# davidfang00/opticalflowdiffusion

Hardware: AMD Instinct MI355X
Metric: UNet denoise steps/sec @ 2x436x1024 flow, bs=16 (higher is better)
Workload: dtype bf16

## Files before the change

### opticalflowdiffusion_amd/csrc/blocks.h

```cpp
#pragma once
#include "common.h"

namespace ofd {

struct MlpDesc {
    const float* weight;
    const float* bias;
    int n_out;
    int offset;
};

struct FcFuse { const float* w; const float* b; float* out; };
bool conv_fc_fuse_supported(const ofd_conv_args* a, int out_dim);
int conv_forward_impl(const ofd_conv_args* a, hipStream_t s, int pool2 = 0, const bf16_t* residual_b = nullptr, const FcFuse* fc = nullptr);
bool conv_pool2_supported(const ofd_conv_args* a);
bool conv_residual_b_supported(const ofd_conv_args* a);
int k_wt_transpose(const bf16_t* w, bf16_t* wt, int taps, int Cin, int Cout, hipStream_t s);
int k_conv_wgrad(const ofd_conv_args* a, const bf16_t* dy, float* dw, hipStream_t s, float* dbias = nullptr);
int k_conv7_wgrad(const bf16_t* x16, const bf16_t* dy, float* dw, int B, int H, int W, hipStream_t s, float* dbias = nullptr, int channels = 16);
int k_channel_sum(const bf16_t* dy, float* out, size_t npix, int C, hipStream_t s);
int k_wgrad_finish(const float* acc, const float* w_raw, float* dst, int Cout, int Cin, int Cin_pad, int ksize, float ws_eps, int unshuffle,
                   int accumulate, hipStream_t s);
int k_grad_scatter(const bf16_t* D, int Ctot, int ch_off, bf16_t* dst, int C, int B, int H, int W, int mode, int p1, int p2, int accumulate,
                   hipStream_t s);

struct ofd_weight_prep_desc {
    const float* w;
    void* out;
    int Cout, Cin, Cin_pad, ksize;
    float ws_eps;
    int unshuffle;
    int block0;
};
int k_conv_weight_prep_batched(const ofd_weight_prep_desc* d_descs, int n, int total_blocks, hipStream_t s);
int k_wt_transpose_batched(const ofd_weight_prep_desc* d_descs, int n, int total_blocks, hipStream_t s);
int k_pack_input(const float* x, int Cx, const float* cond, int Cc, bf16_t* out, int B, int H, int W, hipStream_t s, int cpad = 16, int ax = 0, int ac = 0);
int k_time_mlp(const int64_t* t, const float* w1, const float* b1, const float* w2, const float* b2, float* temb,
               float* temb_silu, int B, int dim, hipStream_t s);
int k_block_mlp(const float* temb_silu, const MlpDesc* descs, int n_desc, float* ss, int B, int tdim, int ss_stride, hipStream_t s);
int k_gn_finalize(const float* partial, int B, int H, int W, int C, const float* gamma, const float* beta, const float* ss,
                  int ss_stride, int ss_offset, float* a_out, float* s_out, hipStream_t s, float* stats_out = nullptr);
int k_resblock_out(const bf16_t* h, const float* a, const float* sft, const bf16_t* x, bf16_t* out, int B, int H, int W, int C, hipStream_t s);
int k_layernorm_c(const bf16_t* x, const float* g, const bf16_t* res, bf16_t* out, size_t npix, int C, float eps, hipStream_t s);
int la_parts(int B, int n);
int k_linear_attention_core(const bf16_t* qkv, float* partial, float* ctx, bf16_t* out, int B, int n, hipStream_t s, float* ml_out = nullptr,
                            const bf16_t* wo = nullptr, const float* bo = nullptr, bf16_t* o2 = nullptr, int C = 0);
int la_fused_blocks(int n, int B, int C = 64);
int la_fwd_parts(int B, int n);
int k_linear_attention_fused_train(const bf16_t* x, const bf16_t* wq, const bf16_t* wkv, const bf16_t* woutp, const float* bias, const float* g_pre,
                                   const float* g2, float* partial, bf16_t* ctxfrag, float* ctx, float* ml, bf16_t* xn, bf16_t* qkv, bf16_t* o2,
                                   bf16_t* y, int B, int n, int C, float eps_pre, float eps_post, hipStream_t s);
int k_la_weight_prep(const float* wqkv, const float* g, const float* wout, bf16_t* wq, bf16_t* wkv, bf16_t* woutp, int C, hipStream_t s);
int k_linear_attention_fused(const bf16_t* x, const bf16_t* wq, const bf16_t* wkv, const bf16_t* woutp, const float* bias, const float* g2,
                             float* partial, bf16_t* ctxfrag, bf16_t* y, int B, int n, int C, float eps_pre, float eps_post, hipStream_t s);
int k_flash_attention(const bf16_t* qkv, bf16_t* out, int B, int n, hipStream_t s, float* lse = nullptr);
int k_final_conv(const bf16_t* x, const float* w, const float* bias, float* out, int B, int H, int W, int C, int out_dim, hipStream_t s, int out_mode = 0,
                 float out_div = 1.0f);
int k_nhwc_to_nchw(const bf16_t* x, float* out, int B, int H, int W, int C, hipStream_t s);
int k_nchw_to_nhwc(const float* x, bf16_t* out, int B, int H, int W, int C, hipStream_t s);

int k_affine_silu(const bf16_t* h, const float* a, const float* s, bf16_t* out, int B, int H, int W, int C, hipStream_t st);
size_t gn_bwd_workspace_floats(int B, int H, int W, int C);
int k_gn_silu_backward(const bf16_t* g, const bf16_t* h, const float* a, const float* s, const float* stats, const float* gamma,
                       const float* beta, const float* ss, int ss_stride, int ss_offset, bf16_t* dh, float* dgamma, float* dbeta, float* dss,
                       float* workspace, int B, int H, int W, int C, hipStream_t st, float* dconv_bias = nullptr);
int k_layernorm_c_bwd(const bf16_t* x, const float* gw, const bf16_t* dy, bf16_t* dx, float* dg, size_t npix, int C, float eps, int accumulate,
                      hipStream_t st, const bf16_t* extra = nullptr);
int k_final_conv_bwd(const bf16_t* x, const float* w, const float* dy, bf16_t* dx, float* dw, float* db, int B, int H, int W, int C, int out_dim,
                     hipStream_t st, const float* bias = nullptr, int out_mode = 0, float out_div = 1.0f);
int k_conv7_dgrad(const bf16_t* dy, const bf16_t* wt, int cin_pad, float* dx, int cx, int B, int H, int W, float scale, hipStream_t s);
int k_block_mlp_bwd(const float* dss, const float* temb_silu, const float* weight, int n_out, int offset, float* dweight, float* dbias, float* dts,
                    int B, int tdim, int ss_stride, hipStream_t st);
int k_time_mlp_bwd(const int64_t* t, const float* temb, const float* dts, const float* w1, const float* b1, const float* w2, float* dw1, float* db1,
                   float* dw2, float* db2, float* scratch, int B, int dim, hipStream_t st);
int k_grad_add(bf16_t* dst, const bf16_t* src, size_t elems, int accumulate, hipStream_t st);

size_t la_bwd_workspace_floats(int B, int n);
int k_linear_attention_core_bwd(const bf16_t* qkv, const bf16_t* dout, const float* ctx, const float* ml, bf16_t* dqkv, float* workspace, int B, int n,
                                hipStream_t s);
int k_linear_attention_block_bwd(const bf16_t* qkv, const bf16_t* do2, const float* ctx, const float* ml, float* workspace, int B, int n, hipStream_t s,
                                 const bf16_t* xn, const bf16_t* wt, float* dw, bf16_t* dxn, const bf16_t* wo_fwd, const bf16_t* wo_t, float* dwo,
                                 float* dbo, const bf16_t* wq);
int k_flash_attention_bwd(const bf16_t* qkv, const bf16_t* o, const bf16_t* dout, const float* lse, bf16_t* dqkv, float* delta, int B, int n,
                          hipStream_t s);

}
```

### opticalflowdiffusion_amd/csrc/la_fused.hip

```cpp
#include <cstdlib>
#include <type_traits>
#include "blocks.h"
#include "la_common.h"

namespace ofd {

template <int C>
struct XRaw {
    u32x4 v[C / 16];
};

template <int C>
__device__ __forceinline__ void load_raw_x(const bf16_t* __restrict__ xrow, XRaw<C>& r, int half) {
#pragma unroll
    for (int s = 0; s < C / 16; ++s) r.v[s] = *(const u32x4*)(xrow + 16 * s + 8 * half);
}

template <int N16, class At>
__device__ __forceinline__ void la_stage(unsigned char* dst, const bf16_t* __restrict__ src, int tid, At at) {
    static_assert(N16 % (8 * 256) == 0, "whole turns of eight units per thread");
    for (int i0 = tid; i0 < N16; i0 += 8 * 256) {
        uint4 v[8];
#pragma unroll
        for (int k = 0; k < 8; ++k) v[k] = ((const uint4*)src)[at(i0 + k * 256)];
#pragma unroll
        for (int k = 0; k < 8; ++k) ((uint4*)dst)[i0 + k * 256] = v[k];
    }
}
template <int N16>
__device__ __forceinline__ void la_stage(unsigned char* dst, const bf16_t* __restrict__ src, int tid) {
    la_stage<N16>(dst, src, tid, [](int i) { return i; });
}

typedef __bf16 la_bf16x2 __attribute__((ext_vector_type(2)));
template <int C>
__device__ __forceinline__ void norm_stats(const XRaw<C>& r, float eps, float& rstd, float& off) {
    const la_bf16x2 one = __builtin_bit_cast(la_bf16x2, 0x3f803f80u);
    float s1 = 0.0f, s2 = 0.0f;
#pragma unroll
    for (int s = 0; s < C / 16; ++s)
#pragma unroll
        for (int j = 0; j < 4; ++j) {
            const la_bf16x2 w = __builtin_bit_cast(la_bf16x2, (uint32_t)r.v[s][j]);
            s1 = __builtin_amdgcn_fdot2_f32_bf16(w, one, s1, false);
            s2 = __builtin_amdgcn_fdot2_f32_bf16(w, w, s2, false);
        }
    s1 += __shfl_xor(s1, 32, 64);
    s2 += __shfl_xor(s2, 32, 64);
    const float mean = s1 * (1.0f / C);
    const float var = fmaxf(__builtin_fmaf(-mean, mean, s2 * (1.0f / C)), 0.0f);
    rstd = rsqrtf(var + eps);
    off = -mean * rstd;
}
template <int C>
__device__ __forceinline__ void norm_x(const XRaw<C>& r, float eps, bf16x8 (&xs)[C / 16]) {
    float rstd, off;
    norm_stats<C>(r, eps, rstd, off);
#pragma unroll
    for (int s = 0; s < C / 16; ++s)
#pragma unroll
        for (int j = 0; j < 4; ++j) {
            const uint32_t w = r.v[s][j];
            xs[s][2 * j] = (__bf16)__builtin_fmaf(bf2f((bf16_t)(w & 0xffffu)), rstd, off);
            xs[s][2 * j + 1] = (__bf16)__builtin_fmaf(bf2f((bf16_t)(w >> 16)), rstd, off);
// ... 56 lines not shown
    }
    __syncthreads();
}

template <int NH>
__device__ __forceinline__ void ctx_state_init(f32x16 (&ctxT)[NH], float (&m)[NH], float (&l)[NH]) {
#pragma unroll
    for (int hd = 0; hd < NH; ++hd) {
        m[hd] = -3.0e38f;
        l[hd] = 0.0f;
#pragma unroll
        for (int r = 0; r < 16; ++r) ctxT[hd][r] = 0.0f;
    }
}
__device__ __forceinline__ f32x16 ctx_mask_rows(f32x16 ka, int tile, int n, int half) {
    if (tile * 32 + 32 > n) {
#pragma unroll
        for (int r = 0; r < 16; ++r)
            if (tile * 32 + acc_row(r, half) >= n) ka[r] = -3.0e38f;
    }
    return ka;
}
__device__ __forceinline__ float ctx_tile_max(const f32x16& ka) {
    float mt = -3.0e38f;
#pragma unroll
    for (int r = 0; r < 16; ++r) mt = fmaxf(mt, ka[r]);
    return fmaxf(mt, __shfl_xor(mt, 32, 64));
}
__device__ __forceinline__ void ctx_update(f32x16& ctxT, const f32x16& va, const f32x16& p) {
#pragma unroll
    for (int s2 = 0; s2 < 2; ++s2) ctxT = __builtin_amdgcn_mfma_f32_32x32x16_bf16(acc_frag(va, s2), acc_frag(p, s2), ctxT, 0, 0, 0);
}

template <int C, bool TRAIN, int HPW = 4>
__global__ void __launch_bounds__(256, C >= 256 ? 1 : 2) la_ctx_fused_kernel(const bf16_t* __restrict__ x, const bf16_t* __restrict__ wkv,
                                                           float* __restrict__ partial, int n, float eps, float defer,
                                                           const float* __restrict__ g, bf16_t* __restrict__ xn_out, bf16_t* __restrict__ qkv_out) {
    extern __shared__ __attribute__((aligned(16))) unsigned char smem[];
    static_assert(HPW == 4 || (HPW == 2 && !TRAIN), "the training form writes all four heads' k | v");
    constexpr int KS = C / 16, WR = 64 * HPW;
    const int tid = threadIdx.x, lane = tid & 63, wave = tid >> 6, l31 = lane & 31, half = lane >> 5;
    const int h0 = HPW == 4 ? 0 : blockIdx.z * HPW;
    if constexpr (C < 256) {
        for (int i = tid; i < (C / 8) * 256; i += 256) ((uint4*)smem)[i] = ((const uint4*)wkv)[i];
    } else {
        la_stage<(C / 8) * WR>(smem, wkv, tid, [&](int i) {
            const int r = i % WR, kv = r / (32 * HPW);
            return (i / WR) * 256 + kv * 128 + h0 * 32 + (r - kv * 32 * HPW);
        });
    }
    float* s_g = (float*)(smem + (C / 8) * WR * 16);
    if constexpr (TRAIN)
        for (int i = tid; i < C; i += 256) s_g[i] = g[i];
    __syncthreads();
    const int b = blockIdx.y, wave_id = blockIdx.x * 4 + wave, nw = gridDim.x * 4, ntiles = (n + 31) / 32;

    f32x16 ctxT[HPW];
    float m[HPW], l[HPW];
    ctx_state_init<HPW>(ctxT, m, l);
    const bf16_t* xb = x + (size_t)b * n * C;
    XRaw<C> raw_next;
    load_raw_x<C>(xb + (size_t)min(wave_id * 32 + l31, n - 1) * C, raw_next, half);
    for (int tile = wave_id; tile < ntiles; tile += nw) {
        asm volatile("" ::: "memory");
        const XRaw<C> raw = raw_next;
        load_raw_x<C>(xb + (size_t)min((tile + nw) * 32 + l31, n - 1) * C, raw_next, half);
        bf16x8 xs[KS];
        const int pix = tile * 32 + l31;
        if constexpr (TRAIN) {
            norm_x_gain<C>(raw, eps, s_g, half, xs);
            if (pix < n) {
                bf16_t* xrow = xn_out + ((size_t)b * n + pix) * C;
#pragma unroll
                for (int s = 0; s < KS; ++s) *(bf16x8*)(xrow + 16 * s + 8 * half) = xs[s];
            }
        } else {
            norm_x<C>(raw, eps, xs);
        }
        if constexpr (TRAIN) {
            bf16_t* qrow = qkv_out + ((size_t)b * n + min(pix, n - 1)) * 384 + 128;
#pragma unroll
            for (int blk = 0; blk < 8; ++blk) {
                f32x16 t;
#pragma unroll
                for (int r = 0; r < 16; ++r) t[r] = 0.0f;
#pragma unroll
                for (int s = 0; s < KS; ++s)
                    t = __builtin_amdgcn_mfma_f32_32x32x16_bf16(*(const bf16x8*)(smem + ((size_t)(2 * s + half) * 256 + blk * 32 + l31) * 16), xs[s], t, 0, 0, 0);
                store_acc_rows(t, qrow + blk * 32, half, pix < n);
            }
        }
#pragma unroll
        for (int hd = 0; hd < HPW; ++hd) {
            f32x16 ka, va;
#pragma unroll
            for (int r = 0; r < 16; ++r) { ka[r] = 0.0f; va[r] = 0.0f; }
#pragma unroll
            for (int s = 0; s < KS; ++s) {
                const bf16x8 wk = *(const bf16x8*)(smem + ((size_t)(2 * s + half) * WR + hd * 32 + l31) * 16);
                const bf16x8 wv = *(const bf16x8*)(smem + ((size_t)(2 * s + half) * WR + 32 * HPW + hd * 32 + l31) * 16);
                ka = __builtin_amdgcn_mfma_f32_32x32x16_bf16(xs[s], wk, ka, 0, 0, 0);
// ... 272 lines not shown
#pragma unroll
            for (int k = 0; k < 2; ++k) {
                const int c0 = rt * 32 + 8 * (g + k) + 4 * half;
                const float4 gv = *(const float4*)(s_g2 + c0);
                const float o0 = acc_o[rt][4 * (g + k)] * rstd * gv.x + bf2f((bf16_t)(xq[k][0] & 0xffffu));
                const float o1 = acc_o[rt][4 * (g + k) + 1] * rstd * gv.y + bf2f((bf16_t)(xq[k][0] >> 16));
                const float o2 = acc_o[rt][4 * (g + k) + 2] * rstd * gv.z + bf2f((bf16_t)(xq[k][1] & 0xffffu));
                const float o3 = acc_o[rt][4 * (g + k) + 3] * rstd * gv.w + bf2f((bf16_t)(xq[k][1] >> 16));
                qo[k] = pack_quad(o0, o1, o2, o3);
            }
            store_quad_pair(yrow + rt * 32 + 8 * g, qo[0], qo[1], half, ok);
        }
}

template <int C, bool TRAIN>
__global__ void __launch_bounds__(256, C == 64 ? 4 : C == 128 ? 2 : 1) la_out_fused_kernel(const bf16_t* __restrict__ x, const bf16_t* __restrict__ wq,
                                                           const bf16_t* __restrict__ woutp, const bf16_t* __restrict__ ctxfrag,
                                                           const float* __restrict__ bias, const float* __restrict__ g2,
                                                           bf16_t* __restrict__ y, int n, float eps_pre, float eps_post, float scale,
                                                           const float* __restrict__ g, bf16_t* __restrict__ o2_out) {
    extern __shared__ __attribute__((aligned(16))) unsigned char smem[];
    constexpr int KS = C / 16, RT = C / 32;
    constexpr int WQ_B = (C / 8) * 128 * 16, WO_B = 16 * C * 16, CF_B = 4 * 2 * 64 * 16;
    unsigned char* s_wq = smem;
    unsigned char* s_wo = smem + WQ_B;
    unsigned char* s_cf = s_wo + WO_B;
    float* s_bias = (float*)(s_cf + CF_B);
    float* s_g2 = s_bias + C;
    float* s_g = s_g2 + C;
    const int tid = threadIdx.x, lane = tid & 63, wave = tid >> 6, l31 = lane & 31, half = lane >> 5;
    const int b = blockIdx.y;
    if constexpr (TRAIN)
        for (int i = tid; i < C; i += 256) s_g[i] = g[i];
    if constexpr (C < 256) {
        for (int i = tid; i < WQ_B / 16; i += 256) ((uint4*)s_wq)[i] = ((const uint4*)wq)[i];
        for (int i = tid; i < WO_B / 16; i += 256) ((uint4*)s_wo)[i] = ((const uint4*)woutp)[i];
    } else {
        la_stage<WQ_B / 16>(s_wq, wq, tid);
        la_stage<WO_B / 16>(s_wo, woutp, tid);
    }
    for (int i = tid; i < CF_B / 16; i += 256) ((uint4*)s_cf)[i] = ((const uint4*)(ctxfrag + (size_t)b * 4096))[i];
    for (int i = tid; i < C; i += 256) { s_bias[i] = bias[i]; s_g2[i] = g2[i]; }
    __syncthreads();
    const int wave_id = blockIdx.x * 4 + wave, nw = gridDim.x * 4, ntiles = (n + 31) / 32;

    const bf16_t* xb = x + (size_t)b * n * C;
    XRaw<C> raw_next;
    load_raw_x<C>(xb + (size_t)min(wave_id * 32 + l31, n - 1) * C, raw_next, half);
    for (int tile = wave_id; tile < ntiles; tile += nw) {
        asm volatile("" ::: "memory");
        const int pix = tile * 32 + l31;
        const size_t row = (size_t)b * n + min(pix, n - 1);
        const XRaw<C> raw = raw_next;
        load_raw_x<C>(xb + (size_t)min((tile + nw) * 32 + l31, n - 1) * C, raw_next, half);
        bf16x8 xs[KS];
        if constexpr (TRAIN) norm_x_gain<C>(raw, eps_pre, s_g, half, xs);
        else norm_x<C>(raw, eps_pre, xs);
        f32x16 acc_o[RT];
#pragma unroll
        for (int rt = 0; rt < RT; ++rt)
#pragma unroll
            for (int r = 0; r < 16; ++r) acc_o[rt][r] = 0.0f;
#pragma unroll
        for (int hd = 0; hd < 4; ++hd) {
            const f32x16 oa = la_head_out<C, TRAIN>(xs, s_wq, s_cf, hd, scale, lane);
#pragma unroll
            for (int s2 = 0; s2 < 2; ++s2) la_to_out<C>(acc_o, acc_frag(oa, s2), s_wo, hd * 2 + s2, l31, half);
        }
        la_out_tail<C, TRAIN>(acc_o, [&](int s) { return raw.v[s]; }, s_bias, s_g2, y + row * C, TRAIN ? o2_out + row * C : nullptr, pix < n, half, eps_post);
    }
}

template <int C>
// ... 80 lines not shown
                                                             bf16_t* __restrict__ wq, bf16_t* __restrict__ wkv, bf16_t* __restrict__ woutp, int C) {
    const int total = 512 * C;
    for (int i = blockIdx.x * blockDim.x + threadIdx.x; i < total; i += gridDim.x * blockDim.x) {
        if (i < 128 * C) {
            const int j = i & 7, o = (i >> 3) & 127, c8 = i >> 10, c = c8 * 8 + j;
            wq[i] = f2bf(wqkv[(size_t)o * C + c] * (g ? g[c] : 1.0f));
        } else if (i < 384 * C) {
            const int k = i - 128 * C;
            const int j = k & 7, o = (k >> 3) & 255, c8 = k >> 11, c = c8 * 8 + j;
            wkv[k] = f2bf(wqkv[(size_t)(128 + o) * C + c] * (g ? g[c] : 1.0f));
        } else if (woutp) {
            const int k = i - 384 * C;
            const int j = k & 7, c = (k >> 3) % C, rest = (k >> 3) / C;
            const int hh = rest & 1, s2 = (rest >> 1) & 1, hd = rest >> 2;
            woutp[k] = f2bf(wout[(size_t)c * 128 + hd * 32 + 16 * s2 + 8 * (j >> 2) + 4 * hh + (j & 3)]);
        }
    }
}

constexpr float LA_DEFER = 5.545177f;
constexpr int LA_GX2_CAP = 128;
static int la_out_blocks(int n, int B, int C) {
    if (C >= 256) {
        const int gx2 = cdiv(cdiv(n, 32), 4), cap2 = 256 / B;
        return gx2 < cap2 ? gx2 : (cap2 < 1 ? 1 : cap2);
    }
    int gx2 = cdiv(cdiv(n, 32), 4 * 4);
    if (gx2 < 1) gx2 = 1;
    const int cap2 = (LA_GX2_CAP * B < 1024) ? 1024 / B : LA_GX2_CAP;
    if (gx2 > cap2) gx2 = cap2;
    return gx2;
}

template <int C>
static int launch_la(const bf16_t* x, const bf16_t* wq, const bf16_t* wkv, const bf16_t* woutp, const float* bias, const float* g2,
                     float* partial, bf16_t* ctxfrag, bf16_t* y, int B, int n, float eps_pre, float eps_post, hipStream_t s) {
    constexpr int HPW = C == 512 ? 2 : 4;
    constexpr bool SPLIT2 = C == 512;
    constexpr int LDS1 = (C / 8) * 64 * HPW * 16;
    constexpr int LDS2 = (C / 8) * 128 * 16 + 16 * C * 16 + 4 * 2 * 64 * 16 + 2 * C * 4;
    constexpr int LDS2H = (C / 8) * 128 * 16 + 4 * 2 * 64 * 16, LDS2T = 16 * C * 16 + 2 * C * 4;
    static_assert(LDS1 <= 160 * 1024 && (SPLIT2 ? LDS2H <= 160 * 1024 && LDS2T <= 160 * 1024 : LDS2 <= 160 * 1024), "the weights of a pass must fit the LDS");
    static bool attr = false;
    if (!attr) {
        OFD_HIP(hipFuncSetAttribute((const void*)la_ctx_fused_kernel<C, false, HPW>, hipFuncAttributeMaxDynamicSharedMemorySize, LDS1));
        if constexpr (SPLIT2) {
            OFD_HIP(hipFuncSetAttribute((const void*)la_heads_kernel<C>, hipFuncAttributeMaxDynamicSharedMemorySize, LDS2H));
            OFD_HIP(hipFuncSetAttribute((const void*)la_tail_kernel<C>, hipFuncAttributeMaxDynamicSharedMemorySize, LDS2T));
        } else {
            OFD_HIP(hipFuncSetAttribute((const void*)la_out_fused_kernel<C, false>, hipFuncAttributeMaxDynamicSharedMemorySize, LDS2));
        }
        attr = true;
    }
    const int gx = la_fused_blocks(n, B, C), gx2 = la_out_blocks(n, B, C);
    la_ctx_fused_kernel<C, false, HPW><<<dim3(gx, B, 4 / HPW), 256, LDS1, s>>>(x, wkv, partial, n, eps_pre, LA_DEFER, nullptr, nullptr, nullptr);
    la_ctx_combine_kernel<<<dim3(B * 4, 4), 256, 0, s>>>(partial, ctxfrag, gx, 1.0f / (float)n, nullptr);
    if constexpr (SPLIT2) {
        la_heads_kernel<C><<<dim3(gx2, B), 256, LDS2H, s>>>(x, wq, ctxfrag, y, n, eps_pre, LA_SCALE);
        la_tail_kernel<C><<<dim3(gx2, B), 256, LDS2T, s>>>(x, woutp, bias, g2, y, n, eps_post);
    } else {
        la_out_fused_kernel<C, false><<<dim3(gx2, B), 256, LDS2, s>>>(x, wq, woutp, ctxfrag, bias, g2, y, n, eps_pre, eps_post, LA_SCALE, nullptr, nullptr);
    }
    OFD_LAUNCH_CHECK();
    return OFD_OK;
}

int k_linear_attention_fused_train(const bf16_t* x, const bf16_t* wq, const bf16_t* wkv, const bf16_t* woutp, const float* bias, const float* g_pre,
                                   const float* g2, float* partial, bf16_t* ctxfrag, float* ctx, float* ml, bf16_t* xn, bf16_t* qkv, bf16_t* o2,
                                   bf16_t* y, int B, int n, int C, float eps_pre, float eps_post, hipStream_t s) {
    if (C != 64) { set_error("linear_attention_fused_train: C=%d unsupported", C); return OFD_ERR_ARG; }
    constexpr int LDS1 = (64 / 8) * 256 * 16 + 64 * 4;
    constexpr int LDS2 = (64 / 8) * 128 * 16 + 16 * 64 * 16 + 4 * 2 * 64 * 16 + 3 * 64 * 4;
    static bool attr = false;
    if (!attr) {
        OFD_HIP(hipFuncSetAttribute((const void*)la_ctx_fused_kernel<64, true>, hipFuncAttributeMaxDynamicSharedMemorySize, LDS1));
        OFD_HIP(hipFuncSetAttribute((const void*)la_out_fused_kernel<64, true>, hipFuncAttributeMaxDynamicSharedMemorySize, LDS2));
        attr = true;
    }
    const int gx = la_fused_blocks(n, B);
    la_ctx_fused_kernel<64, true><<<dim3(gx, B), 256, LDS1, s>>>(x, wkv, partial, n, eps_pre, LA_DEFER, g_pre, xn, qkv);
    la_ctx_combine_kernel<<<dim3(B * 4, 4), 256, 0, s>>>(partial, ctxfrag, gx, 1.0f / (float)n, nullptr);
    launch_la_ctx_combine(partial, ctx, B, gx, 1.0f / (float)n, ml, s);
    la_out_fused_kernel<64, true><<<dim3(la_out_blocks(n, B, 64), B), 256, LDS2, s>>>(x, wq, woutp, ctxfrag, bias, g2, y, n, eps_pre, eps_post, LA_SCALE, g_pre, o2);
    OFD_LAUNCH_CHECK();
    return OFD_OK;
}

int la_fused_blocks(int n, int B, int C) {
    constexpr int total = 256;
    int gx = cdiv(cdiv(n, 32), 8);
    int cap = total / (B < 1 ? 1 : B);
    if (C >= 256) cap = (cap < 32 ? 32 : cap) / (C / 256);
    else if (cap < 64) cap = 64;
    if (cap < 1) cap = 1;
    if (gx < 1) gx = 1;
    if (gx > cap) gx = cap;
    return gx;
}

int k_la_weight_prep(const float* wqkv, const float* g, const float* wout, bf16_t* wq, bf16_t* wkv, bf16_t* woutp, int C, hipStream_t s) {
    la_weight_prep_kernel<<<cdiv((woutp ? 512 : 384) * C, 256), 256, 0, s>>>(wqkv, g, wout, wq, wkv, woutp, C);
    OFD_LAUNCH_CHECK();
    return OFD_OK;
}

int k_linear_attention_fused(const bf16_t* x, const bf16_t* wq, const bf16_t* wkv, const bf16_t* woutp, const float* bias, const float* g2,
                             float* partial, bf16_t* ctxfrag, bf16_t* y, int B, int n, int C, float eps_pre, float eps_post, hipStream_t s) {
    if (C == 64) return launch_la<64>(x, wq, wkv, woutp, bias, g2, partial, ctxfrag, y, B, n, eps_pre, eps_post, s);
    if (C == 128) return launch_la<128>(x, wq, wkv, woutp, bias, g2, partial, ctxfrag, y, B, n, eps_pre, eps_post, s);
    if (C == 256) return launch_la<256>(x, wq, wkv, woutp, bias, g2, partial, ctxfrag, y, B, n, eps_pre, eps_post, s);
    if (C == 512) return launch_la<512>(x, wq, wkv, woutp, bias, g2, partial, ctxfrag, y, B, n, eps_pre, eps_post, s);
    set_error("linear_attention_fused: C=%d unsupported", C);
    return OFD_ERR_ARG;
}

}
```

### opticalflowdiffusion_amd/csrc/unet.hip

```cpp
#include <cstdlib>
#include "unet_exec.h"

using namespace ofd;

namespace ofd {

float site_eps(const ofd_unet* u, const std::string& site) {
    if (u->cfg.eps_mode == 0) return 1e-5f;
    auto ends = [&](const char* s) { std::string t(s); return site.size() >= t.size() && site.compare(site.size() - t.size(), t.size(), t) == 0; };
    if (ends(".fn.fn.to_out.1")) return 1e-3f;
    if (ends(".0.block1.proj") && site.rfind("downs.", 0) == 0) return 1e-3f;
    if (site == "mid_block1.block1.proj" || site == "final_res_block.block1.proj") return 1e-3f;
    return 1e-5f;
}

static void add_param(ofd_unet* u, const std::string& name, std::vector<int> shape) {
    size_t numel = 1;
    for (int d : shape) numel *= (size_t)d;
    Param p{name, (int)shape.size(), {1, 1, 1, 1}, numel, u->n_param_floats, false};
    for (size_t i = 0; i < shape.size(); ++i) p.shape[i] = shape[i];
    u->pindex[name] = (int)u->params.size();
    u->params.push_back(p);
    u->n_param_floats += (numel + 3) / 4 * 4;
}
// ... 92 lines not shown
    if (c.rc != OFD_OK) return;
    const ConvDesc& d = c.u->convs[c.u->cindex.at(prefix)];
    ofd_conv_args a{};
    a.B = c.B; a.H = out.H; a.W = out.W; a.ksize = d.ksize; a.n_src = (int)srcs.size(); a.Cout = d.Cout;
    int cin = 0;
    for (size_t i = 0; i < srcs.size(); ++i) {
        a.src[i].src = srcs[i].t.p;
        a.src[i].channels = srcs[i].t.C;
        a.src[i].src_channels = srcs[i].t.C;
        a.src[i].ch_offset = 0;
        a.src[i].upsample = srcs[i].upsample;
        a.src[i].unshuffle = srcs[i].unshuffle;
        a.src[i].p1 = srcs[i].p1;
        a.src[i].p2 = srcs[i].p2;
        cin += srcs[i].t.C;
    }
    const bool pack8 = d.ksize == 7 && cin == 8 && d.pack8_off >= 0;
    if (cin != d.Cin_pad && !pack8) { set_error("conv %s: got %d input channels, expected %d", prefix.c_str(), cin, d.Cin_pad); c.rc = OFD_ERR_ARG; return; }
    a.weight = c.u->d_wbuf + (pack8 ? (size_t)d.pack8_off : d.w_off);
    a.bias = c.u->P(prefix + ".bias");
    a.in_scale = in_scale; a.in_shift = in_shift; a.residual = residual; a.res_act = res_act;
    a.res_scale = res_scale; a.res_shift = res_shift; a.out = out.p; a.gn_partial = gn_partial;
    const double px = (double)c.B * out.H * out.W;
    const double flops = 2.0 * px * d.Cout * (double)d.Cin * d.ksize * d.ksize;
    const double bytes = px * 2.0 * (d.Cout + (double)cin / ((srcs[0].upsample) ? 4 : 1)) + (double)d.ksize * d.ksize * d.Cin_pad * d.Cout * 2.0;
    const bool pp = d.ksize == 3 && d.Cout == 64 && cin == 64 && srcs.size() == 1 && !srcs[0].upsample && !residual && !res_act;
    const int cls3 = pp ? PC_CONV3_PP : (d.Cout % 128 == 0 ? PC_CONV3 : PC_CONV3_64);
    c.begin(d.ksize == 3 ? cls3 : (d.ksize == 1 ? PC_CONV1 : PC_CONV7), flops, bytes,
            prefix + " " + std::to_string(d.Cin) + "->" + std::to_string(d.Cout) + " @" + std::to_string(out.H) + "x" + std::to_string(out.W));
    RUN(conv_forward_impl(&a, c.s, 0, nullptr, fc));
    c.end();
}

static Tensor resblock(Ctx& c, const std::string& name, const std::vector<Tensor>& in, int Cout, bool keep_out = true, const FcFuse* fc = nullptr) {
    ofd_unet* u = c.u;
    const int H = in[0].H, W = in[0].W, B = c.B;
    std::vector<SrcSpec> srcs;
    int cin = 0;
    for (auto& t : in) { SrcSpec s; s.t = t; srcs.push_back(s); cin += t.C; }
    Tensor h1 = c.tmp(Cout, H, W), h2 = c.tmp(Cout, H, W);
    const size_t np = ofd_conv_gn_partial_count(B, H, W, Cout);
    float* p1 = c.tmpf(np);
    float* p2 = c.tmpf(np);
    float* a1 = c.train ? c.keepf((size_t)B * Cout) : c.tmpf((size_t)B * Cout);
    float* s1 = c.train ? c.keepf((size_t)B * Cout) : c.tmpf((size_t)B * Cout);
    float* a2 = c.train ? c.keepf((size_t)B * Cout) : c.tmpf((size_t)B * Cout);
    float* s2 = c.train ? c.keepf((size_t)B * Cout) : c.tmpf((size_t)B * Cout);
    float* st1 = c.train ? c.keepf((size_t)B * 16) : nullptr;
    float* st2 = c.train ? c.keepf((size_t)B * 16) : nullptr;
    Tensor out = keep_out ? c.keep(Cout, H, W) : c.tmp(Cout, H, W);
    if (c.rc != OFD_OK) return out;
    conv(c, name + ".block1.proj", srcs, h1, nullptr, nullptr, nullptr, nullptr, nullptr, nullptr, p1);
    c.begin(PC_GN, 0, (double)np * 4);
    RUN(k_gn_finalize(p1, B, H, W, Cout, u->P(name + ".block1.norm.weight"), u->P(name + ".block1.norm.bias"), c.ss, u->ss_stride,
                      u->ss_offset.at(name), a1, s1, c.s, st1));
    c.end();
    SrcSpec hs; hs.t = h1;
    constexpr int act1_min = 256;
    constexpr int act1_train_min = 128;
    const int amin = c.train ? act1_train_min : act1_min;
    Tensor act1;
    if (Cout >= amin) {
        act1 = c.tmp(Cout, H, W);
        if (c.rc != OFD_OK) return out;
        c.begin(PC_MISC, 0, (double)B * H * W * Cout * 4.0);
        RUN(k_affine_silu(h1.p, a1, s1, act1.p, B, H, W, Cout, c.s));
        c.end();
        hs.t = act1;
        conv(c, name + ".block2.proj", {hs}, h2, nullptr, nullptr, nullptr, nullptr, nullptr, nullptr, p2);
    } else
    conv(c, name + ".block2.proj", {hs}, h2, a1, s1, nullptr, nullptr, nullptr, nullptr, p2);
    c.begin(PC_GN, 0, (double)np * 4);
    RUN(k_gn_finalize(p2, B, H, W, Cout, u->P(name + ".block2.norm.weight"), u->P(name + ".block2.norm.bias"), nullptr, 0, 0, a2, s2, c.s, st2));
    c.end();
    if (cin != Cout) {
        conv(c, name + ".res_conv", srcs, out, nullptr, nullptr, nullptr, h2.p, a2, s2, nullptr, fc);
    } else {
        c.begin(PC_RESOUT, 0, (double)B * H * W * Cout * 6.0);
        RUN(k_resblock_out(h2.p, a2, s2, in[0].p, out.p, B, H, W, Cout, c.s));
        c.end();
    }
    if (c.train) {
        TapeRec r;
        r.kind = TK_RES; r.name = name; r.srcs = srcs; r.out = out; r.h1 = h1; r.h2 = h2;
        r.a1 = a1; r.s1 = s1; r.a2 = a2; r.s2 = s2; r.st1 = st1; r.st2 = st2; r.act1 = act1;
        u->tape.push_back(r);
    }
    return out;
}

static Tensor linattn(Ctx& c, const std::string& name, Tensor x) {
    ofd_unet* u = c.u;
    const int H = x.H, W = x.W, B = c.B, C = x.C, n = H * W;
    const size_t npix = (size_t)B * n;
    auto fit = u->la_fused.find(name);
    if (fit != u->la_fused.end() && !c.train && (C <= 128 || env_int("OFD_LA_FUSED_WIDE", 1))) {
        const int nparts = la_fused_blocks(n, B, C);
        float* partial = c.tmpf((size_t)B * 4 * nparts * 1088);
        bf16_t* ctxfrag = (bf16_t*)c.tmpf((size_t)B * 2048);
        Tensor y = c.keep(C, H, W);
        if (c.rc != OFD_OK) return y;
        const bf16_t* base = u->d_labuf + fit->second.first;
        c.begin(PC_LINATTN, npix * 2.0 * (C * 384.0 + 2 * 4 * 32 * 32 + 128.0 * C), (double)npix * C * 2 * 3,
                name + " fused C=" + std::to_string(C) + " @" + std::to_string(H) + "x" + std::to_string(W));
        RUN(k_linear_attention_fused(x.p, base, base + (size_t)128 * C, base + (size_t)384 * C, u->P(name + ".fn.fn.to_out.0.bias"),
                                     u->P(name + ".fn.fn.to_out.1.g"), partial, ctxfrag, y.p, B, n, C, site_eps(u, name + ".fn.norm"),
                                     site_eps(u, name + ".fn.fn.to_out.1"), c.s));
        c.end();
        return y;
    }
    Tensor xn = c.tmp(C, H, W), qkv = c.tmp(384, H, W), ao = c.tmp(128, H, W), o2 = c.tmp(C, H, W);
    const int nparts = la_fwd_parts(B, n);
    if (c.train && fit != u->la_fused.end() && la_train_fused(C)) {
        float* partial = c.tmpf((size_t)B * 4 * nparts * 1088);
        bf16_t* ctxfrag = (bf16_t*)c.tmpf((size_t)B * 2048);
        float* ctx = c.keepf((size_t)B * 4 * 1024);
        float* ml = c.keepf((size_t)B * 4 * 64);
        Tensor y = c.keep(C, H, W);
        if (c.rc != OFD_OK) return y;
        const bf16_t* base = u->d_labuf + fit->second.first;
        c.begin(PC_LINATTN, npix * 2.0 * (C * 640.0 + 2 * 4 * 32 * 32 + 128.0 * C), (double)npix * C * 2 * (2 + 1 + 4 + 2),
                name + " fused (training) C=" + std::to_string(C) + " @" + std::to_string(H) + "x" + std::to_string(W));
        RUN(k_linear_attention_fused_train(x.p, base + (size_t)512 * C, base + (size_t)640 * C, base + (size_t)384 * C, u->P(name + ".fn.fn.to_out.0.bias"),
                                           u->P(name + ".fn.norm.g"), u->P(name + ".fn.fn.to_out.1.g"), partial, ctxfrag, ctx, ml, xn.p, qkv.p, o2.p, y.p,
                                           B, n, C, site_eps(u, name + ".fn.norm"), site_eps(u, name + ".fn.fn.to_out.1"), c.s));
        c.end();
        TapeRec r;
        r.kind = TK_LINATTN; r.name = name; r.x = x; r.xn = xn; r.qkv = qkv; r.ao = ao; r.o2 = o2; r.out = y; r.ctx = ctx; r.ml = ml;
        u->tape.push_back(r);
        return y;
    }
    float* partial = c.tmpf((size_t)B * 4 * nparts * 1088);
    float* ctx = c.train ? c.keepf((size_t)B * 4 * 1024) : c.tmpf((size_t)B * 4 * 1024);
    float* ml = c.train ? c.keepf((size_t)B * 4 * 64) : nullptr;
    Tensor y = c.keep(C, H, W);
    if (c.rc != OFD_OK) return y;
    c.begin(PC_LN, 0, (double)npix * C * 4);
    RUN(k_layernorm_c(x.p, u->P(name + ".fn.norm.g"), nullptr, xn.p, npix, C, site_eps(u, name + ".fn.norm"), c.s));
    c.end();
    SrcSpec s; s.t = xn;
// ... 85 lines not shown
int run_forward(Ctx& c, const float* x, int Cx, const float* cond, int Cc, const int64_t* t, float* out, int H, int W, float* temb,
                float* temb_silu) {
    ofd_unet* u = c.u;
    const int B = c.B, dim = u->cfg.dim;
    u->taps.clear();
    u->last_B = B;
    if (c.train) u->tape.clear();
    const bool pack8 = u->convs[u->cindex.at("init_conv")].pack8_off >= 0;
    const int cpad = pack8 ? 8 : u->cin_pad;
    const int L = u->L;
    Tensor xin = c.keep(cpad, H, W);
    c.begin(PC_MISC, 0, 0);
    RUN(k_pack_input(x, Cx, cond, cond ? Cc : 0, xin.p, B, H, W, c.s, cpad, u->glue_x, u->glue_cond));
    if (!u->cfg.no_time) {
        RUN(k_time_mlp(t, u->P("time_mlp.1.weight"), u->P("time_mlp.1.bias"), u->P("time_mlp.3.weight"), u->P("time_mlp.3.bias"), temb, temb_silu, B, dim, c.s));
        RUN(k_block_mlp(temb_silu, u->d_mlp, (int)u->resblocks.size(), c.ss, B, dim * 4, u->ss_stride, c.s));
    } else {
        c.ss = nullptr;
    }
    c.end();
    Tensor r = c.keep(dim, H, W);
    { SrcSpec s; s.t = xin; plain_conv(c, "init_conv", {s}, r); }
    u->taps["init_conv"] = r;

    Tensor xcur = r;
    std::vector<Tensor> hs;
    for (int i = 0; i < L; ++i) {
        const std::string p = "downs." + std::to_string(i);
        c.reset_scratch();
        xcur = resblock(c, p + ".0", {xcur}, u->dims[i]);
        hs.push_back(xcur);
        u->taps[p + ".0"] = xcur;
        c.reset_scratch();
        Tensor x1 = resblock(c, p + ".1", {xcur}, u->dims[i]);
        u->taps[p + ".1"] = x1;
        c.reset_scratch();
        xcur = linattn(c, p + ".2", x1);
        hs.push_back(xcur);
        u->taps[p + ".2"] = xcur;
        if (i < L - 1) {
            Tensor d = c.keep(u->dims[i + 1], xcur.H / 2, xcur.W / 2);
            std::vector<SrcSpec> srcs;
            for (int sub = 0; sub < 4; ++sub) { SrcSpec s; s.t = xcur; s.unshuffle = 1; s.p1 = sub >> 1; s.p2 = sub & 1; srcs.push_back(s); }
            plain_conv(c, p + ".3.1", srcs, d);
            xcur = d;
        } else {
            Tensor d = c.keep(u->dims[i + 1], xcur.H, xcur.W);
            SrcSpec s; s.t = xcur;
            plain_conv(c, p + ".3", {s}, d);
            xcur = d;
        }
        u->taps[p + ".3"] = xcur;
    }
    c.reset_scratch();
    xcur = resblock(c, "mid_block1", {xcur}, u->dims[L]);
    u->taps["mid_block1"] = xcur;
    c.reset_scratch();
    xcur = midattn(c, xcur);
    u->taps["mid_attn"] = xcur;
    c.reset_scratch();
    xcur = resblock(c, "mid_block2", {xcur}, u->dims[L]);
    u->taps["mid_block2"] = xcur;
    for (int i = 0; i < L; ++i) {
        const std::string p = "ups." + std::to_string(i);
        const int co = u->dims[L - i], ci = u->dims[L - 1 - i];
        c.reset_scratch();
        Tensor h = hs.back(); hs.pop_back();
        xcur = resblock(c, p + ".0", {xcur, h}, co);
        u->taps[p + ".0"] = xcur;
        c.reset_scratch();
// ... 510 lines not shown
```

### opticalflowdiffusion_amd/csrc/unet_exec.h

```cpp
#pragma once
#include <cstdlib>
#include <array>
#include <map>
#include <tuple>
#include <string>
#include <vector>
#include "blocks.h"
#include "det.h"

namespace ofd {

struct Param {
    std::string name;
    int ndim;
    int shape[4];
    size_t numel;
    size_t offset;
    bool set;
};

struct ConvDesc {
    std::string wname;
    int Cout, Cin, Cin_pad, ksize;
    float ws_eps;
// ... 146 lines not shown
    size_t grad_offset = 0;
    size_t scratch_high = 0;

    void* alloc(char* base, size_t& used, size_t cap, size_t bytes) {
        bytes = (bytes + 255) / 256 * 256;
        if (used + bytes > cap) {
            if (rc == OFD_OK) { set_error("unet_forward: workspace too small"); rc = OFD_ERR_WORKSPACE; }
            return nullptr;
        }
        void* p = base + used;
        used += bytes;
        if (base == scratch && used > scratch_high) scratch_high = used;
        return p;
    }
    Tensor keep(int C, int H, int W) {
        Tensor t;
        t.p = (bf16_t*)alloc(persist, persist_used, persist_cap, (size_t)B * H * W * C * 2);
        t.C = C; t.H = H; t.W = W;
        if (train && t.p) t.g = (bf16_t*)((char*)t.p + grad_offset);
        return t;
    }
    float* keepf(size_t n) { return (float*)alloc(persist, persist_used, persist_cap, n * 4); }
    Tensor tmp(int C, int H, int W) {
        if (train) return keep(C, H, W);
        Tensor t;
        t.p = (bf16_t*)alloc(scratch, scratch_used, scratch_cap, (size_t)B * H * W * C * 2);
        t.C = C; t.H = H; t.W = W;
        return t;
    }
    float* tmpf(size_t n) { return (float*)alloc(scratch, scratch_used, scratch_cap, n * 4); }
    int blocks_done = 0, signal_at = -1;
    hipEvent_t signal_ev = nullptr;
    bool signalled = false;
    void reset_scratch() {
        scratch_used = 0;
        if (signal_ev && !signalled && !dry && blocks_done++ >= signal_at) { (void)hipEventRecord(signal_ev, s); signalled = true; }
    }

    bool in_region = false, chain_ok = false;
    hipEvent_t last_end = nullptr;
    hipEvent_t next_event() {
        while (u->pool.size() < u->pool_used + 1) {
            hipEvent_t e;
            if (hipEventCreate(&e) != hipSuccess) return nullptr;
            u->pool.push_back(e);
        }
        return u->pool[u->pool_used++];
    }
    void begin(int cls, double flops, double bytes, const std::string& label = std::string()) {
        if (!u->profiling || dry) return;
        hipEvent_t e0 = chain_ok ? last_end : next_event();
        hipEvent_t e1 = next_event();
        if (!e0 || !e1) return;
        ProfRec r{cls, e0, e1, flops, bytes, label};
        if (!chain_ok) (void)hipEventRecord(r.e0, s);
        u->recs.push_back(r);
        in_region = true;
    }
    void end() {
        if (!u->profiling || dry || u->recs.empty() || !in_region) return;
        (void)hipEventRecord(u->recs.back().e1, s);
        last_end = u->recs.back().e1;
        chain_ok = true;
        in_region = false;
    }
};

static inline bool la_train_fused(int C) { return C == 64; }
// ... 24 lines not shown
```

Measured before the change: 35.09.

## Fuse resblock output epilogue into linear-attention context kernel at C=64

```diff
diff --git a/opticalflowdiffusion_amd/csrc/blocks.h b/opticalflowdiffusion_amd/csrc/blocks.h
--- a/opticalflowdiffusion_amd/csrc/blocks.h
+++ b/opticalflowdiffusion_amd/csrc/blocks.h
@@ -51,8 +51,17 @@
                                    const float* g2, float* partial, bf16_t* ctxfrag, float* ctx, float* ml, bf16_t* xn, bf16_t* qkv, bf16_t* o2,
                                    bf16_t* y, int B, int n, int C, float eps_pre, float eps_post, hipStream_t s);
 int k_la_weight_prep(const float* wqkv, const float* g, const float* wout, bf16_t* wq, bf16_t* wkv, bf16_t* woutp, int C, hipStream_t s);
+struct LaTail {
+    const bf16_t* h;
+    const float* a;
+    const float* s;
+    const bf16_t* x_in;
+    bf16_t* out;
+};
+bool la_tail_supported(int C);
 int k_linear_attention_fused(const bf16_t* x, const bf16_t* wq, const bf16_t* wkv, const bf16_t* woutp, const float* bias, const float* g2,
-                             float* partial, bf16_t* ctxfrag, bf16_t* y, int B, int n, int C, float eps_pre, float eps_post, hipStream_t s);
+                             float* partial, bf16_t* ctxfrag, bf16_t* y, int B, int n, int C, float eps_pre, float eps_post, hipStream_t s,
+                             const LaTail* tail = nullptr);
 int k_flash_attention(const bf16_t* qkv, bf16_t* out, int B, int n, hipStream_t s, float* lse = nullptr);
 int k_final_conv(const bf16_t* x, const float* w, const float* bias, float* out, int B, int H, int W, int C, int out_dim, hipStream_t s, int out_mode = 0,
                  float out_div = 1.0f);
diff --git a/opticalflowdiffusion_amd/csrc/la_fused.hip b/opticalflowdiffusion_amd/csrc/la_fused.hip
--- a/opticalflowdiffusion_amd/csrc/la_fused.hip
+++ b/opticalflowdiffusion_amd/csrc/la_fused.hip
@@ -1,6 +1,7 @@
 #include <cstdlib>
 #include <type_traits>
 #include "blocks.h"
+#include "conv_common.h"
 #include "la_common.h"
 
 namespace ofd {
@@ -18,18 +19,37 @@
 
 template <int N16, class At>
 __device__ __forceinline__ void la_stage(unsigned char* dst, const bf16_t* __restrict__ src, int tid, At at) {
-    static_assert(N16 % (8 * 256) == 0, "whole turns of eight units per thread");
-    for (int i0 = tid; i0 < N16; i0 += 8 * 256) {
-        uint4 v[8];
-#pragma unroll
-        for (int k = 0; k < 8; ++k) v[k] = ((const uint4*)src)[at(i0 + k * 256)];
-#pragma unroll
-        for (int k = 0; k < 8; ++k) ((uint4*)dst)[i0 + k * 256] = v[k];
+    constexpr int U = N16 >= 8 * 256 ? 8 : N16 / 256;
+    static_assert(U >= 1 && N16 % (U * 256) == 0, "whole turns of U units per thread");
+    for (int i0 = tid; i0 < N16; i0 += U * 256) {
+        uint4 v[U];
+#pragma unroll
+        for (int k = 0; k < U; ++k) v[k] = ((const uint4*)src)[at(i0 + k * 256)];
+#pragma unroll
+        for (int k = 0; k < U; ++k) ((uint4*)dst)[i0 + k * 256] = v[k];
     }
 }
 template <int N16>
 __device__ __forceinline__ void la_stage(unsigned char* dst, const bf16_t* __restrict__ src, int tid) {
     la_stage<N16>(dst, src, tid, [](int i) { return i; });
+}
+
+template <int C>
+__device__ __forceinline__ void resblock_tail(const XRaw<C>& h, const XRaw<C>& xin, const float* __restrict__ a, const float* __restrict__ sft, int half,
+                                              XRaw<C>& o) {
+#pragma unroll
+    for (int s = 0; s < C / 16; ++s) {
+        const float4 a0 = *(const float4*)(a + 16 * s + 8 * half), a1 = *(const float4*)(a + 16 * s + 8 * half + 4);
+        const float4 s0 = *(const float4*)(sft + 16 * s + 8 * half), s1 = *(const float4*)(sft + 16 * s + 8 * half + 4);
+        const float av[8] = {a0.x, a0.y, a0.z, a0.w, a1.x, a1.y, a1.z, a1.w}, sv[8] = {s0.x, s0.y, s0.z, s0.w, s1.x, s1.y, s1.z, s1.w};
+#pragma unroll
+        for (int j = 0; j < 4; ++j) {
+            const uint32_t hw = h.v[s][j], xw = xin.v[s][j];
+            const float lo = silu_f(bf2f((bf16_t)(hw & 0xffffu)) * av[2 * j] + sv[2 * j]) + bf2f((bf16_t)(xw & 0xffffu));
+            const float hi = silu_f(bf2f((bf16_t)(hw >> 16)) * av[2 * j + 1] + sv[2 * j + 1]) + bf2f((bf16_t)(xw >> 16));
+            o.v[s][j] = f2bf2(lo, hi);
+        }
+    }
 }
 
 typedef __bf16 la_bf16x2 __attribute__((ext_vector_type(2)));
@@ -152,17 +172,19 @@
     for (int s2 = 0; s2 < 2; ++s2) ctxT = __builtin_amdgcn_mfma_f32_32x32x16_bf16(acc_frag(va, s2), acc_frag(p, s2), ctxT, 0, 0, 0);
 }
 
-template <int C, bool TRAIN, int HPW = 4>
+template <int C, bool TRAIN, int HPW = 4, bool TAIL = false>
 __global__ void __launch_bounds__(256, C >= 256 ? 1 : 2) la_ctx_fused_kernel(const bf16_t* __restrict__ x, const bf16_t* __restrict__ wkv,
                                                            float* __restrict__ partial, int n, float eps, float defer,
-                                                           const float* __restrict__ g, bf16_t* __restrict__ xn_out, bf16_t* __restrict__ qkv_out) {
+                                                           const float* __restrict__ g, bf16_t* __restrict__ xn_out, bf16_t* __restrict__ qkv_out,
+                                                           LaTail tail) {
     extern __shared__ __attribute__((aligned(16))) unsigned char smem[];
     static_assert(HPW == 4 || (HPW == 2 && !TRAIN), "the training form writes all four heads' k | v");
+    static_assert(!TAIL || (!TRAIN && HPW == 4), "the tail form: inference, one workgroup for all heads (a row of x has one writer)");
     constexpr int KS = C / 16, WR = 64 * HPW;
     const int tid = threadIdx.x, lane = tid & 63, wave = tid >> 6, l31 = lane & 31, half = lane >> 5;
     const int h0 = HPW == 4 ? 0 : blockIdx.z * HPW;
     if constexpr (C < 256) {
-        for (int i = tid; i < (C / 8) * 256; i += 256) ((uint4*)smem)[i] = ((const uint4*)wkv)[i];
+        la_stage<(C / 8) * 256>(smem, wkv, tid);
     } else {
         la_stage<(C / 8) * WR>(smem, wkv, tid, [&](int i) {
             const int r = i % WR, kv = r / (32 * HPW);
@@ -170,23 +192,39 @@
         });
     }
     float* s_g = (float*)(smem + (C / 8) * WR * 16);
+    const int b = blockIdx.y, wave_id = blockIdx.x * 4 + wave, nw = gridDim.x * 4, ntiles = (n + 31) / 32;
     if constexpr (TRAIN)
         for (int i = tid; i < C; i += 256) s_g[i] = g[i];
-    __syncthreads();
-    const int b = blockIdx.y, wave_id = blockIdx.x * 4 + wave, nw = gridDim.x * 4, ntiles = (n + 31) / 32;
+    if constexpr (TAIL)
+        for (int i = tid; i < 2 * C; i += 256) s_g[i] = i < C ? tail.a[(size_t)b * C + i] : tail.s[(size_t)b * C + i - C];
+    __syncthreads();
 
     f32x16 ctxT[HPW];
     float m[HPW], l[HPW];
     ctx_state_init<HPW>(ctxT, m, l);
-    const bf16_t* xb = x + (size_t)b * n * C;
-    XRaw<C> raw_next;
+    const bf16_t* __restrict__ xb = (TAIL ? tail.h : x) + (size_t)b * n * C;
+    const bf16_t* __restrict__ rb = TAIL ? tail.x_in + (size_t)b * n * C : nullptr;
+    XRaw<C> raw_next, res_next;
     load_raw_x<C>(xb + (size_t)min(wave_id * 32 + l31, n - 1) * C, raw_next, half);
+    if constexpr (TAIL) load_raw_x<C>(rb + (size_t)min(wave_id * 32 + l31, n - 1) * C, res_next, half);
     for (int tile = wave_id; tile < ntiles; tile += nw) {
         asm volatile("" ::: "memory");
-        const XRaw<C> raw = raw_next;
-        load_raw_x<C>(xb + (size_t)min((tile + nw) * 32 + l31, n - 1) * C, raw_next, half);
+        XRaw<C> raw = raw_next;
+        const int pix = tile * 32 + l31;
+        if constexpr (TAIL) {
+            const XRaw<C> res = res_next;
+            load_raw_x<C>(xb + (size_t)min((tile + nw) * 32 + l31, n - 1) * C, raw_next, half);
+            load_raw_x<C>(rb + (size_t)min((tile + nw) * 32 + l31, n - 1) * C, res_next, half);
+            resblock_tail<C>(raw, res, s_g, s_g + C, half, raw);
+            if (pix < n) {
+                bf16_t* orow = tail.out + ((size_t)b * n + pix) * C;
+#pragma unroll
+                for (int s = 0; s < KS; ++s) *(u32x4*)(orow + 16 * s + 8 * half) = raw.v[s];
+            }
+        } else {
+            load_raw_x<C>(xb + (size_t)min((tile + nw) * 32 + l31, n - 1) * C, raw_next, half);
+        }
         bf16x8 xs[KS];
-        const int pix = tile * 32 + l31;
         if constexpr (TRAIN) {
             norm_x_gain<C>(raw, eps, s_g, half, xs);
             if (pix < n) {
@@ -525,13 +563,8 @@
     const int b = blockIdx.y;
     if constexpr (TRAIN)
         for (int i = tid; i < C; i += 256) s_g[i] = g[i];
-    if constexpr (C < 256) {
-        for (int i = tid; i < WQ_B / 16; i += 256) ((uint4*)s_wq)[i] = ((const uint4*)wq)[i];
-        for (int i = tid; i < WO_B / 16; i += 256) ((uint4*)s_wo)[i] = ((const uint4*)woutp)[i];
-    } else {
-        la_stage<WQ_B / 16>(s_wq, wq, tid);
-        la_stage<WO_B / 16>(s_wo, woutp, tid);
-    }
+    la_stage<WQ_B / 16>(s_wq, wq, tid);
+    la_stage<WO_B / 16>(s_wo, woutp, tid);
     for (int i = tid; i < CF_B / 16; i += 256) ((uint4*)s_cf)[i] = ((const uint4*)(ctxfrag + (size_t)b * 4096))[i];
     for (int i = tid; i < C; i += 256) { s_bias[i] = bias[i]; s_g2[i] = g2[i]; }
     __syncthreads();
@@ -678,9 +711,12 @@
     return gx2;
 }
 
+static constexpr bool la_tail_width(int C) { return C == 64; }
+bool la_tail_supported(int C) { return la_tail_width(C); }
+
 template <int C>
 static int launch_la(const bf16_t* x, const bf16_t* wq, const bf16_t* wkv, const bf16_t* woutp, const float* bias, const float* g2,
-                     float* partial, bf16_t* ctxfrag, bf16_t* y, int B, int n, float eps_pre, float eps_post, hipStream_t s) {
+                     float* partial, bf16_t* ctxfrag, bf16_t* y, int B, int n, float eps_pre, float eps_post, hipStream_t s, const LaTail* tail) {
     constexpr int HPW = C == 512 ? 2 : 4;
     constexpr bool SPLIT2 = C == 512;
     constexpr int LDS1 = (C / 8) * 64 * HPW * 16;
@@ -699,7 +735,22 @@
         attr = true;
     }
     const int gx = la_fused_blocks(n, B, C), gx2 = la_out_blocks(n, B, C);
-    la_ctx_fused_kernel<C, false, HPW><<<dim3(gx, B, 4 / HPW), 256, LDS1, s>>>(x, wkv, partial, n, eps_pre, LA_DEFER, nullptr, nullptr, nullptr);
+    if (tail) {
+        if constexpr (la_tail_width(C)) {
+            constexpr int LDS1T = LDS1 + 2 * C * 4;
+            static bool attr_t = false;
+            if (!attr_t) {
+                OFD_HIP(hipFuncSetAttribute((const void*)la_ctx_fused_kernel<C, false, 4, true>, hipFuncAttributeMaxDynamicSharedMemorySize, LDS1T));
+                attr_t = true;
+            }
+            x = tail->out;
+            la_ctx_fused_kernel<C, false, 4, true><<<dim3(gx, B), 256, LDS1T, s>>>(nullptr, wkv, partial, n, eps_pre, LA_DEFER, nullptr, nullptr, nullptr, *tail);
+        } else {
+            set_error("linear_attention_fused: no tail form at C=%d", C);
+            return OFD_ERR_ARG;
+        }
+    } else
+    la_ctx_fused_kernel<C, false, HPW><<<dim3(gx, B, 4 / HPW), 256, LDS1, s>>>(x, wkv, partial, n, eps_pre, LA_DEFER, nullptr, nullptr, nullptr, LaTail{});
     la_ctx_combine_kernel<<<dim3(B * 4, 4), 256, 0, s>>>(partial, ctxfrag, gx, 1.0f / (float)n, nullptr);
     if constexpr (SPLIT2) {
         la_heads_kernel<C><<<dim3(gx2, B), 256, LDS2H, s>>>(x, wq, ctxfrag, y, n, eps_pre, LA_SCALE);
@@ -724,7 +775,7 @@
         attr = true;
     }
     const int gx = la_fused_blocks(n, B);
-    la_ctx_fused_kernel<64, true><<<dim3(gx, B), 256, LDS1, s>>>(x, wkv, partial, n, eps_pre, LA_DEFER, g_pre, xn, qkv);
+    la_ctx_fused_kernel<64, true><<<dim3(gx, B), 256, LDS1, s>>>(x, wkv, partial, n, eps_pre, LA_DEFER, g_pre, xn, qkv, LaTail{});
     la_ctx_combine_kernel<<<dim3(B * 4, 4), 256, 0, s>>>(partial, ctxfrag, gx, 1.0f / (float)n, nullptr);
     launch_la_ctx_combine(partial, ctx, B, gx, 1.0f / (float)n, ml, s);
     la_out_fused_kernel<64, true><<<dim3(la_out_blocks(n, B, 64), B), 256, LDS2, s>>>(x, wq, woutp, ctxfrag, bias, g2, y, n, eps_pre, eps_post, LA_SCALE, g_pre, o2);
@@ -751,11 +802,12 @@
 }
 
 int k_linear_attention_fused(const bf16_t* x, const bf16_t* wq, const bf16_t* wkv, const bf16_t* woutp, const float* bias, const float* g2,
-                             float* partial, bf16_t* ctxfrag, bf16_t* y, int B, int n, int C, float eps_pre, float eps_post, hipStream_t s) {
-    if (C == 64) return launch_la<64>(x, wq, wkv, woutp, bias, g2, partial, ctxfrag, y, B, n, eps_pre, eps_post, s);
-    if (C == 128) return launch_la<128>(x, wq, wkv, woutp, bias, g2, partial, ctxfrag, y, B, n, eps_pre, eps_post, s);
-    if (C == 256) return launch_la<256>(x, wq, wkv, woutp, bias, g2, partial, ctxfrag, y, B, n, eps_pre, eps_post, s);
-    if (C == 512) return launch_la<512>(x, wq, wkv, woutp, bias, g2, partial, ctxfrag, y, B, n, eps_pre, eps_post, s);
+                             float* partial, bf16_t* ctxfrag, bf16_t* y, int B, int n, int C, float eps_pre, float eps_post, hipStream_t s,
+                             const LaTail* tail) {
+    if (C == 64) return launch_la<64>(x, wq, wkv, woutp, bias, g2, partial, ctxfrag, y, B, n, eps_pre, eps_post, s, tail);
+    if (C == 128) return launch_la<128>(x, wq, wkv, woutp, bias, g2, partial, ctxfrag, y, B, n, eps_pre, eps_post, s, tail);
+    if (C == 256) return launch_la<256>(x, wq, wkv, woutp, bias, g2, partial, ctxfrag, y, B, n, eps_pre, eps_post, s, tail);
+    if (C == 512) return launch_la<512>(x, wq, wkv, woutp, bias, g2, partial, ctxfrag, y, B, n, eps_pre, eps_post, s, tail);
     set_error("linear_attention_fused: C=%d unsupported", C);
     return OFD_ERR_ARG;
 }
diff --git a/opticalflowdiffusion_amd/csrc/unet.hip b/opticalflowdiffusion_amd/csrc/unet.hip
--- a/opticalflowdiffusion_amd/csrc/unet.hip
+++ b/opticalflowdiffusion_amd/csrc/unet.hip
@@ -148,7 +148,8 @@
     c.end();
 }
 
-static Tensor resblock(Ctx& c, const std::string& name, const std::vector<Tensor>& in, int Cout, bool keep_out = true, const FcFuse* fc = nullptr) {
+static Tensor resblock(Ctx& c, const std::string& name, const std::vector<Tensor>& in, int Cout, bool keep_out = true, const FcFuse* fc = nullptr,
+                       LaTail* tail = nullptr) {
     ofd_unet* u = c.u;
     const int H = in[0].H, W = in[0].W, B = c.B;
     std::vector<SrcSpec> srcs;
@@ -191,6 +192,8 @@
     c.end();
     if (cin != Cout) {
         conv(c, name + ".res_conv", srcs, out, nullptr, nullptr, nullptr, h2.p, a2, s2, nullptr, fc);
+    } else if (tail) {
+        *tail = LaTail{h2.p, a2, s2, in[0].p, out.p};
     } else {
         c.begin(PC_RESOUT, 0, (double)B * H * W * Cout * 6.0);
         RUN(k_resblock_out(h2.p, a2, s2, in[0].p, out.p, B, H, W, Cout, c.s));
@@ -205,7 +208,11 @@
     return out;
 }
 
-static Tensor linattn(Ctx& c, const std::string& name, Tensor x) {
+static bool la_tail_fuse(const Ctx& c, const std::string& la_name, int C) {
+    return !c.train && c.u->la_fused.count(la_name) && la_tail_supported(C) && env_int("OFD_LA_TAIL_FUSE", 1);
+}
+
+static Tensor linattn(Ctx& c, const std::string& name, Tensor x, const LaTail* tail = nullptr) {
     ofd_unet* u = c.u;
     const int H = x.H, W = x.W, B = c.B, C = x.C, n = H * W;
     const size_t npix = (size_t)B * n;
@@ -217,11 +224,11 @@
         Tensor y = c.keep(C, H, W);
         if (c.rc != OFD_OK) return y;
         const bf16_t* base = u->d_labuf + fit->second.first;
-        c.begin(PC_LINATTN, npix * 2.0 * (C * 384.0 + 2 * 4 * 32 * 32 + 128.0 * C), (double)npix * C * 2 * 3,
-                name + " fused C=" + std::to_string(C) + " @" + std::to_string(H) + "x" + std::to_string(W));
-        RUN(k_linear_attention_fused(x.p, base, base + (size_t)128 * C, base + (size_t)384 * C, u->P(name + ".fn.fn.to_out.0.bias"),
+        c.begin(PC_LINATTN, npix * 2.0 * (C * 384.0 + 2 * 4 * 32 * 32 + 128.0 * C), (double)npix * C * 2 * (tail ? 5 : 3),
+                name + (tail ? " fused + tail C=" : " fused C=") + std::to_string(C) + " @" + std::to_string(H) + "x" + std::to_string(W));
+        RUN(k_linear_attention_fused(tail ? nullptr : x.p, base, base + (size_t)128 * C, base + (size_t)384 * C, u->P(name + ".fn.fn.to_out.0.bias"),
                                      u->P(name + ".fn.fn.to_out.1.g"), partial, ctxfrag, y.p, B, n, C, site_eps(u, name + ".fn.norm"),
-                                     site_eps(u, name + ".fn.fn.to_out.1"), c.s));
+                                     site_eps(u, name + ".fn.fn.to_out.1"), c.s, tail));
         c.end();
         return y;
     }
@@ -373,10 +380,12 @@
         hs.push_back(xcur);
         u->taps[p + ".0"] = xcur;
         c.reset_scratch();
-        Tensor x1 = resblock(c, p + ".1", {xcur}, u->dims[i]);
+        LaTail tail;
+        const bool fuse_tail = la_tail_fuse(c, p + ".2", u->dims[i]);
+        Tensor x1 = resblock(c, p + ".1", {xcur}, u->dims[i], true, nullptr, fuse_tail ? &tail : nullptr);
         u->taps[p + ".1"] = x1;
-        c.reset_scratch();
-        xcur = linattn(c, p + ".2", x1);
+        c.reset_scratch(fuse_tail);
+        xcur = linattn(c, p + ".2", x1, fuse_tail ? &tail : nullptr);
         hs.push_back(xcur);
         u->taps[p + ".2"] = xcur;
         if (i < L - 1) {
diff --git a/opticalflowdiffusion_amd/csrc/unet_exec.h b/opticalflowdiffusion_amd/csrc/unet_exec.h
--- a/opticalflowdiffusion_amd/csrc/unet_exec.h
+++ b/opticalflowdiffusion_amd/csrc/unet_exec.h
@@ -202,8 +202,8 @@
     int blocks_done = 0, signal_at = -1;
     hipEvent_t signal_ev = nullptr;
     bool signalled = false;
-    void reset_scratch() {
-        scratch_used = 0;
+    void reset_scratch(bool keep = false) {
+        if (!keep) scratch_used = 0;
         if (signal_ev && !signalled && !dry && blocks_done++ >= signal_at) { (void)hipEventRecord(signal_ev, s); signalled = true; }
     }
 
```

Result: no change. 35.42 (median of 6 runs) (+0.9%).
